# cgranerob/Land-Surface-Temperature-Super-Resolution-with-a-Scale-Invariance-Free-Neural-Approach

Measured on AMD Instinct MI355X. Metric: LST+NDVI 256x256 patches/sec (train fwd+bwd), whole job, higher is better.
Workload: dtype f32; 1 GPU; ModelB SIF-NN-SR2 (gradFTM loss) batch 64/GPU, synthetic 256x256, 1x MI355X, fwd+loss+bwd+Adam; batch_per_gpu=64, patch=256x256 (LST 64x64 + NDVI 256x256), parallelism=dp1, loss=sr2

## Files before the change

land-surface-temperature-super-resolution-with-a-scale-invariance-free-neural-approach_amd/csrc/resample.hip:

```cpp
#include "edge_conv.h"

namespace {

__device__ __forceinline__ float4 maybe_bnrelu(float4 v, const float* scale, const float* shift, int c) {
  return scale != nullptr ? bn_relu4(v, ld4(scale + c), ld4(shift + c)) : v;
}

template <bool HS>
__global__ void bnrelu_pool2_kernel(const float* __restrict__ y, const float* scale, const float* shift,
                                    float* __restrict__ out, int B, int H, int W, int C) {
  const unsigned Q = C / 4, Ho = H / 2, Wo = W / 2;
  const unsigned n = (unsigned)B * Ho * Wo * Q;
  for (unsigned e = blockIdx.x * blockDim.x + threadIdx.x; e < n; e += gridDim.x * blockDim.x) {
    const unsigned p = e / Q;
    const int c = (int)(e - p * Q) * 4;
    const unsigned rr = p / Wo, ox = p - rr * Wo, b = rr / Ho, oy = rr - b * Ho;
    const size_t s = (((size_t)b * H + 2 * oy) * W + 2 * ox) * C + c;
    const float4 v00 = maybe_bnrelu(ldA4<HS>(y, s), scale, shift, c), v01 = maybe_bnrelu(ldA4<HS>(y, s + C), scale, shift, c);
    const float4 v10 = maybe_bnrelu(ldA4<HS>(y, s + (size_t)W * C), scale, shift, c);
    const float4 v11 = maybe_bnrelu(ldA4<HS>(y, s + (size_t)W * C + C), scale, shift, c);
    float4 o;
    o.x = (v00.x + v01.x + v10.x + v11.x) * 0.25f;
    o.y = (v00.y + v01.y + v10.y + v11.y) * 0.25f;
    o.z = (v00.z + v01.z + v10.z + v11.z) * 0.25f;
    o.w = (v00.w + v01.w + v10.w + v11.w) * 0.25f;
    stA4<HS>(out, (size_t)p * C + c, o);
  }
}

template <bool HS>
__global__ void bnrelu_add_kernel(const float* __restrict__ p, const float* __restrict__ y, const float* scale,
                                  const float* shift, float* __restrict__ out, int C, size_t nquads) {
  const unsigned Q = C / 4;
  for (size_t e = (size_t)blockIdx.x * blockDim.x + threadIdx.x; e < nquads; e += (size_t)gridDim.x * blockDim.x) {
    const int c = (int)((unsigned)e % Q) * 4;
    const float4 a = ldA4<HS>(p, e * 4), v = maybe_bnrelu(ldA4<HS>(y, e * 4), scale, shift, c);
    stA4<HS>(out, e * 4, make_float4(a.x + v.x, a.y + v.y, a.z + v.z, a.w + v.w));
  }
}

__device__ __forceinline__ void up_coord(int o, int in, int out, int& i0, int& i1, float& l0, float& l1) {
  const float ratio = out > 1 ? (float)(in - 1) / (float)(out - 1) : 0.f;
  const float src = ratio * (float)o;
  i0 = (int)src;
  i1 = i0 + (i0 < in - 1 ? 1 : 0);
  l1 = src - (float)i0;
  l0 = 1.f - l1;
}

template <bool HS>
__global__ void bnrelu_up2x_kernel(const float* __restrict__ y, const float* scale, const float* shift,
                                   float* __restrict__ out, int B, int Hin, int Win, int C) {
  const int Q = C / 4, Ho = 2 * Hin, Wo = 2 * Win;
  const size_t n = (size_t)B * Ho * Wo * Q;
  for (size_t e = (size_t)blockIdx.x * blockDim.x + threadIdx.x; e < n; e += (size_t)gridDim.x * blockDim.x) {
    const int c = (int)(e % Q) * 4;
    const size_t p = e / Q;
    const int ox = p % Wo, oy = (p / Wo) % Ho, b = p / ((size_t)Wo * Ho);
    int y0, y1, x0, x1; float hy0, hy1, hx0, hx1;
    up_coord(oy, Hin, Ho, y0, y1, hy0, hy1);
    up_coord(ox, Win, Wo, x0, x1, hx0, hx1);
    const size_t base = (size_t)b * Hin * Win * C + c;
    const float4 v00 = maybe_bnrelu(ldA4<HS>(y, base + ((size_t)y0 * Win + x0) * C), scale, shift, c);
    const float4 v01 = maybe_bnrelu(ldA4<HS>(y, base + ((size_t)y0 * Win + x1) * C), scale, shift, c);
    const float4 v10 = maybe_bnrelu(ldA4<HS>(y, base + ((size_t)y1 * Win + x0) * C), scale, shift, c);
    const float4 v11 = maybe_bnrelu(ldA4<HS>(y, base + ((size_t)y1 * Win + x1) * C), scale, shift, c);
    float4 o;
    o.x = hy0 * (hx0 * v00.x + hx1 * v01.x) + hy1 * (hx0 * v10.x + hx1 * v11.x);
    o.y = hy0 * (hx0 * v00.y + hx1 * v01.y) + hy1 * (hx0 * v10.y + hx1 * v11.y);
    o.z = hy0 * (hx0 * v00.z + hx1 * v01.z) + hy1 * (hx0 * v10.z + hx1 * v11.z);
    o.w = hy0 * (hx0 * v00.w + hx1 * v01.w) + hy1 * (hx0 * v10.w + hx1 * v11.w);
    stA4<HS>(out, p * C + c, o);
  }
}

template <bool HS>
__global__ void pool2_bwd_kernel(const float* __restrict__ gp, float* __restrict__ g, int B, int H, int W, int C,
                                 int accumulate) {
  const int Q = C / 4, Ho = H / 2, Wo = W / 2;
  const size_t n = (size_t)B * H * W * Q;
  for (size_t e = (size_t)blockIdx.x * blockDim.x + threadIdx.x; e < n; e += (size_t)gridDim.x * blockDim.x) {
    const int c = (int)(e % Q) * 4;
    const size_t p = e / Q;
    const int x = p % W, yy = (p / W) % H, b = p / ((size_t)W * H);
    const float4 v = ldA4<HS>(gp, (((size_t)b * Ho + yy / 2) * Wo + x / 2) * C + c);
    float4 o = make_float4(0.25f * v.x, 0.25f * v.y, 0.25f * v.z, 0.25f * v.w);
    if (accumulate) {
      const float4 a = ldA4<HS>(g, p * C + c);
      o.x += a.x; o.y += a.y; o.z += a.z; o.w += a.w;
    }
    stA4<HS>(g, p * C + c, o);
  }
}

template <bool HS>
__global__ void up2x_bwd_kernel(const float* __restrict__ gu, float* __restrict__ g, int B, int Hin, int Win, int C) {
  SIFSR_CHAIN_PRIO();
  const int Q = C / 4, Ho = 2 * Hin, Wo = 2 * Win;
  const size_t n = (size_t)B * Hin * Win * Q;
  for (size_t e = (size_t)blockIdx.x * blockDim.x + threadIdx.x; e < n; e += (size_t)gridDim.x * blockDim.x) {
    const int c = (int)(e % Q) * 4;
    const size_t p = e / Q;
    const int ix = p % Win, iy = (p / Win) % Hin, b = p / ((size_t)Win * Hin);
    float wy[5], wx[5];
#pragma unroll
    for (int k = 0; k < 5; ++k) {
      const int oy = 2 * iy - 2 + k, ox = 2 * ix - 2 + k;
      wy[k] = 0.f; wx[k] = 0.f;
      if (oy >= 0 && oy < Ho) {
        int a0, a1; float l0, l1;
        up_coord(oy, Hin, Ho, a0, a1, l0, l1);
        wy[k] = (a0 == iy ? l0 : 0.f) + (a1 == iy ? l1 : 0.f);
      }
      if (ox >= 0 && ox < Wo) {
        int a0, a1; float l0, l1;
        up_coord(ox, Win, Wo, a0, a1, l0, l1);
        wx[k] = (a0 == ix ? l0 : 0.f) + (a1 == ix ? l1 : 0.f);
      }
    }
    float4 acc = make_float4(0.f, 0.f, 0.f, 0.f);
#pragma unroll
    for (int ky = 0; ky < 5; ++ky) {
      if (wy[ky] == 0.f) continue;
      const int oy = 2 * iy - 2 + ky;
#pragma unroll
      for (int kx = 0; kx < 5; ++kx) {
        if (wx[kx] == 0.f) continue;
        const int ox = 2 * ix - 2 + kx;
        const float w = wy[ky] * wx[kx];
        const float4 v = ldA4<HS>(gu, (((size_t)b * Ho + oy) * Wo + ox) * C + c);
        acc.x = fmaf(w, v.x, acc.x); acc.y = fmaf(w, v.y, acc.y); acc.z = fmaf(w, v.z, acc.z); acc.w = fmaf(w, v.w, acc.w);
      }
    }
    stA4<HS>(g, p * C + c, acc);
  }
}

template <int C, bool HS>
__global__ __launch_bounds__(256) void bnrelu_up2x_tile_kernel(const float* __restrict__ y, const float* scale,
                                                               const float* shift, float* __restrict__ out, int Hin,
                                                               int Win) {
  constexpr int Q = C / 4, SR = 10;
  __shared__ float4 src[SR * SR * Q];
  const int tid = threadIdx.x;
  const int Ho = 2 * Hin, Wo = 2 * Win;
  const int ox0 = blockIdx.x * 16, oy0 = blockIdx.y * 16, b = blockIdx.z;
  int sy0, sx0, t1; float f0, f1;
  up_coord(oy0, Hin, Ho, sy0, t1, f0, f1);
  up_coord(ox0, Win, Wo, sx0, t1, f0, f1);
  for (int e = tid; e < SR * SR * Q; e += 256) {
    const int c4 = e % Q, p = e / Q;
    const int py = p / SR, px = p - py * SR;
    const int gy = min(sy0 + py, Hin - 1), gx = min(sx0 + px, Win - 1);
    src[e] = maybe_bnrelu(ldA4<HS>(y, ((size_t)(b * Hin + gy) * Win + gx) * C + 4 * c4), scale, shift, 4 * c4);
  }
  __syncthreads();
  for (int e = tid; e < 256 * Q; e += 256) {
    const int c4 = e % Q, p = e / Q;
    const int oy = oy0 + (p >> 4), ox = ox0 + (p & 15);
    if (oy >= Ho || ox >= Wo) continue;
    int y0, y1, x0, x1; float hy0, hy1, hx0, hx1;
    up_coord(oy, Hin, Ho, y0, y1, hy0, hy1);
    up_coord(ox, Win, Wo, x0, x1, hx0, hx1);
    const float4 v00 = src[((y0 - sy0) * SR + (x0 - sx0)) * Q + c4], v01 = src[((y0 - sy0) * SR + (x1 - sx0)) * Q + c4];
    const float4 v10 = src[((y1 - sy0) * SR + (x0 - sx0)) * Q + c4], v11 = src[((y1 - sy0) * SR + (x1 - sx0)) * Q + c4];
    float4 o;
    o.x = hy0 * (hx0 * v00.x + hx1 * v01.x) + hy1 * (hx0 * v10.x + hx1 * v11.x);
    o.y = hy0 * (hx0 * v00.y + hx1 * v01.y) + hy1 * (hx0 * v10.y + hx1 * v11.y);
    o.z = hy0 * (hx0 * v00.z + hx1 * v01.z) + hy1 * (hx0 * v10.z + hx1 * v11.z);
    o.w = hy0 * (hx0 * v00.w + hx1 * v01.w) + hy1 * (hx0 * v10.w + hx1 * v11.w);
    stA4<HS>(out, ((size_t)(b * Ho + oy) * Wo + ox) * C + 4 * c4, o);
  }
}

template <int C, bool HS>
__global__ __launch_bounds__(256) void up2x_bwd_tile_kernel(const float* __restrict__ gu, float* __restrict__ g, int Hin,
                                                            int Win, const float* __restrict__ bn_y,
                                                            const float* __restrict__ bn_scale,
                                                            const float* __restrict__ bn_shift,
                                                            float* __restrict__ bn_partials) {
  SIFSR_CHAIN_PRIO();
  constexpr int TL = 8, HR = 2 * TL + 3, NCH = C / 16;
  __shared__ float4 hi[HR * HR * 4];
  __shared__ float4 tmp[HR * TL * 4];
  __shared__ float wxs[TL][5], wys[TL][5];
  const int tid = threadIdx.x;
  const int Ho = 2 * Hin, Wo = 2 * Win;
  const int ix0 = blockIdx.x * TL, iy0 = blockIdx.y * TL;
  const int b = blockIdx.z / NCH, ch0 = (blockIdx.z % NCH) * 16;
  if (tid < 2 * TL * 5) {
    const bool isy = tid >= TL * 5;
    const int t = isy ? tid - TL * 5 : tid;
    const int il = t / 5, k = t - il * 5;
    const int i = (isy ? iy0 : ix0) + il, in = isy ? Hin : Win, on = isy ? Ho : Wo;
    const int o = 2 * i - 2 + k;
    float w = 0.f;
    if (i < in && o >= 0 && o < on) {
      int a0, a1; float l0, l1;
      up_coord(o, in, on, a0, a1, l0, l1);
      w = (a0 == i ? l0 : 0.f) + (a1 == i ? l1 : 0.f);
    }
    if (isy) wys[il][k] = w; else wxs[il][k] = w;
  }
  for (int e = tid; e < HR * HR * 4; e += 256) {
    const int q = e & 3, p = e >> 2;
    const int py = p / HR, px = p - py * HR;
    const int oy = 2 * iy0 - 2 + py, ox = 2 * ix0 - 2 + px;
    float4 v = make_float4(0.f, 0.f, 0.f, 0.f);
    if (oy >= 0 && oy < Ho && ox >= 0 && ox < Wo) v = ldA4<HS>(gu, ((size_t)(b * Ho + oy) * Wo + ox) * C + ch0 + 4 * q);
    hi[e] = v;
  }
  __syncthreads();
  for (int e = tid; e < HR * TL * 4; e += 256) {
    const int q = e & 3, p = e >> 2;
    const int py = p / TL, il = p - py * TL;
    float4 acc = make_float4(0.f, 0.f, 0.f, 0.f);
#pragma unroll
    for (int k = 0; k < 5; ++k) {
      const float w = wxs[il][k];
      const float4 v = hi[(py * HR + 2 * il + k) * 4 + q];
      acc.x = fmaf(w, v.x, acc.x); acc.y = fmaf(w, v.y, acc.y); acc.z = fmaf(w, v.z, acc.z); acc.w = fmaf(w, v.w, acc.w);
    }
    tmp[e] = acc;
  }
  __syncthreads();
  {
    const int q = tid & 3, p = tid >> 2;
    const int il_y = p / TL, il_x = p - il_y * TL;
    const int iy = iy0 + il_y, ix = ix0 + il_x;
    float4 acc = make_float4(0.f, 0.f, 0.f, 0.f);
#pragma unroll
    for (int k = 0; k < 5; ++k) {
      const float w = wys[il_y][k];
      const float4 v = tmp[((2 * il_y + k) * TL + il_x) * 4 + q];
      acc.x = fmaf(w, v.x, acc.x); acc.y = fmaf(w, v.y, acc.y); acc.z = fmaf(w, v.z, acc.z); acc.w = fmaf(w, v.w, acc.w);
    }
    const bool in = iy < Hin && ix < Win;
    acc = as_stored4<HS>(acc);
    if (in) stA4<HS>(g, ((size_t)(b * Hin + iy) * Win + ix) * C + ch0 + 4 * q, acc);
    if (bn_partials != nullptr) {
      float4 d1 = make_float4(0.f, 0.f, 0.f, 0.f), d2 = d1;
      if (in) {
        const float4 yv = ldA4<HS>(bn_y, ((size_t)(b * Hin + iy) * Win + ix) * C + ch0 + 4 * q);
        const float4 sc = ld4(bn_scale + ch0 + 4 * q), sh = ld4(bn_shift + ch0 + 4 * q);
        d1.x = fmaf(yv.x, sc.x, sh.x) > 0.f ? acc.x : 0.f; d2.x = d1.x * yv.x;
        d1.y = fmaf(yv.y, sc.y, sh.y) > 0.f ? acc.y : 0.f; d2.y = d1.y * yv.y;
        d1.z = fmaf(yv.z, sc.z, sh.z) > 0.f ? acc.z : 0.f; d2.z = d1.z * yv.z;
        d1.w = fmaf(yv.w, sc.w, sh.w) > 0.f ? acc.w : 0.f; d2.w = d1.w * yv.w;
      }
      float v8[8] = {d1.x, d1.y, d1.z, d1.w, d2.x, d2.y, d2.z, d2.w};
#pragma unroll
      for (int m = 4; m < 64; m <<= 1)
#pragma unroll
        for (int j = 0; j < 8; ++j) v8[j] += __shfl_xor(v8[j], m);
      __syncthreads();
      float* const red = reinterpret_cast<float*>(hi);
      if ((tid & 63) < 4) {
#pragma unroll
        for (int j = 0; j < 8; ++j) red[((tid >> 6) * 4 + (tid & 3)) * 8 + j] = v8[j];
      }
      __syncthreads();
      if (tid < 32) {
        const int qq = tid & 3, r = (tid >> 2) & 3, which = tid >> 4;
        const float sum = (red[(0 * 4 + qq) * 8 + which * 4 + r] + red[(1 * 4 + qq) * 8 + which * 4 + r]) +
                          (red[(2 * 4 + qq) * 8 + which * 4 + r] + red[(3 * 4 + qq) * 8 + which * 4 + r]);
        const size_t row = ((size_t)b * gridDim.y + blockIdx.y) * gridDim.x + blockIdx.x;
        bn_partials[(row * C + ch0 + 4 * qq + r) * 2 + which] = sum;
      }
    }
  }
}

inline int grid_for(size_t n) {
  size_t b = (n + 255) / 256;
  return (int)(b > 16384 ? 16384 : (b < 1 ? 1 : b));
}

}

int launch_bnrelu_pool2(const float* y, const float* scale, const float* shift, float* out, int B, int H, int W, int C, hipStream_t s) {
  if (H % 2 || W % 2 || C % 4 || (size_t)B * H * W * C >= ((size_t)1 << 32)) return SIFSR_ERR_SHAPE;
  if (sifsr_half_storage()) hipLaunchKernelGGL(bnrelu_pool2_kernel<true>, dim3(grid_for((size_t)B * H / 2 * W / 2 * C / 4)), dim3(256), 0, s, y, scale, shift, out, B, H, W, C);
  else hipLaunchKernelGGL(bnrelu_pool2_kernel<false>, dim3(grid_for((size_t)B * H / 2 * W / 2 * C / 4)), dim3(256), 0, s, y, scale, shift, out, B, H, W, C);
  SIFSR_LAUNCH_CHECK();
  return SIFSR_OK;
}
int launch_bnrelu_add(const float* p, const float* y, const float* scale, const float* shift, float* out, int C, size_t npix, hipStream_t s) {
  if (C % 4) return SIFSR_ERR_SHAPE;
  const size_t nq = npix * C / 4;
  if (sifsr_half_storage()) hipLaunchKernelGGL(bnrelu_add_kernel<true>, dim3(grid_for(nq)), dim3(256), 0, s, p, y, scale, shift, out, C, nq);
  else hipLaunchKernelGGL(bnrelu_add_kernel<false>, dim3(grid_for(nq)), dim3(256), 0, s, p, y, scale, shift, out, C, nq);
  SIFSR_LAUNCH_CHECK();
  return SIFSR_OK;
}
int launch_bnrelu_up2x(const float* y, const float* scale, const float* shift, float* out, int B, int Hin, int Win, int C, hipStream_t s) {
  if (C % 4) return SIFSR_ERR_SHAPE;
  if ((C == 16 || C == 32 || C == 64) && B <= 65535 && Hin >= 2 && Win >= 2) {
    const dim3 grid((2 * Win + 15) / 16, (2 * Hin + 15) / 16, B);
#define SIFSR_UP(CV, HV) hipLaunchKernelGGL((bnrelu_up2x_tile_kernel<CV, HV>), grid, dim3(256), 0, s, y, scale, shift, out, Hin, Win)
    const bool hs = sifsr_half_storage();
    if (C == 16) { if (hs) SIFSR_UP(16, true); else SIFSR_UP(16, false); }
    else if (C == 32) { if (hs) SIFSR_UP(32, true); else SIFSR_UP(32, false); }
    else { if (hs) SIFSR_UP(64, true); else SIFSR_UP(64, false); }
#undef SIFSR_UP
    SIFSR_LAUNCH_CHECK();
    return SIFSR_OK;
  }
  if (sifsr_half_storage()) hipLaunchKernelGGL(bnrelu_up2x_kernel<true>, dim3(grid_for((size_t)B * Hin * Win * C)), dim3(256), 0, s, y, scale, shift, out, B, Hin, Win, C);
  else hipLaunchKernelGGL(bnrelu_up2x_kernel<false>, dim3(grid_for((size_t)B * Hin * Win * C)), dim3(256), 0, s, y, scale, shift, out, B, Hin, Win, C);
  SIFSR_LAUNCH_CHECK();
  return SIFSR_OK;
}
int launch_pool2_bwd(const float* gp, float* g, int B, int H, int W, int C, int accumulate, hipStream_t s) {
  if (H % 2 || W % 2 || C % 4) return SIFSR_ERR_SHAPE;
  if (sifsr_half_storage()) hipLaunchKernelGGL(pool2_bwd_kernel<true>, dim3(grid_for((size_t)B * H * W * C / 4)), dim3(256), 0, s, gp, g, B, H, W, C, accumulate);
  else hipLaunchKernelGGL(pool2_bwd_kernel<false>, dim3(grid_for((size_t)B * H * W * C / 4)), dim3(256), 0, s, gp, g, B, H, W, C, accumulate);
  SIFSR_LAUNCH_CHECK();
  return SIFSR_OK;
}
int up2x_bwd_stat_rows(int B, int Hin, int Win, int C) {
  if (!((C == 16 || C == 32 || C == 64) && (size_t)B * (C / 16) <= 65535)) return 0;
  return B * ((Hin + 7) / 8) * ((Win + 7) / 8);
}

int launch_up2x_bwd(const float* gu, float* g, int B, int Hin, int Win, int C, hipStream_t s, const float* bn_y,
                    const float* bn_scale, const float* bn_shift, float* bn_partials) {
  if (C % 4) return SIFSR_ERR_SHAPE;
  if (bn_partials != nullptr && (!bn_y || !bn_scale || !bn_shift || up2x_bwd_stat_rows(B, Hin, Win, C) == 0)) return SIFSR_ERR_ARG;
  if ((C == 16 || C == 32 || C == 64) && (size_t)B * (C / 16) <= 65535) {
    const dim3 grid((Win + 7) / 8, (Hin + 7) / 8, B * (C / 16));
#define SIFSR_UPB(CV, HV) hipLaunchKernelGGL((up2x_bwd_tile_kernel<CV, HV>), grid, dim3(256), 0, s, gu, g, Hin, Win, bn_y, bn_scale, bn_shift, bn_partials)
    const bool hs = sifsr_half_storage();
    if (C == 16) { if (hs) SIFSR_UPB(16, true); else SIFSR_UPB(16, false); }
    else if (C == 32) { if (hs) SIFSR_UPB(32, true); else SIFSR_UPB(32, false); }
    else { if (hs) SIFSR_UPB(64, true); else SIFSR_UPB(64, false); }
#undef SIFSR_UPB
    SIFSR_LAUNCH_CHECK();
    return SIFSR_OK;
  }
  if (sifsr_half_storage()) hipLaunchKernelGGL(up2x_bwd_kernel<true>, dim3(grid_for((size_t)B * Hin * Win * C / 4)), dim3(256), 0, s, gu, g, B, Hin, Win, C);
  else hipLaunchKernelGGL(up2x_bwd_kernel<false>, dim3(grid_for((size_t)B * Hin * Win * C / 4)), dim3(256), 0, s, gu, g, B, Hin, Win, C);
  SIFSR_LAUNCH_CHECK();
  return SIFSR_OK;
}
```

Baseline: 10680 patches/s.

## Replace tiled up2x backward with register-streaming row-band kernel using wave shuffles

Swaps the shared-memory 8x8 tile kernel for the bilinear-upsample backward pass for one that streams output rows down a band of input rows. Each lane keeps its columns in registers, gets horizontal halo neighbours through wave shuffles, and prefetches several rows ahead. It accumulates two vertical input rows as it goes and fuses the BN statistics partials into the same stream. This removes the LDS staging, the block barriers and the redundant halo loads of the tiled version, in exchange for more register pressure and a different grid and partials layout.

```diff
diff --git a/land-surface-temperature-super-resolution-with-a-scale-invariance-free-neural-approach_amd/csrc/resample.hip b/land-surface-temperature-super-resolution-with-a-scale-invariance-free-neural-approach_amd/csrc/resample.hip
--- a/land-surface-temperature-super-resolution-with-a-scale-invariance-free-neural-approach_amd/csrc/resample.hip
+++ b/land-surface-temperature-super-resolution-with-a-scale-invariance-free-neural-approach_amd/csrc/resample.hip
@@ -173,100 +173,137 @@
   }
 }
 
+constexpr int UPB_PF = 3;
+constexpr int upb_band(int C) { return C == 64 ? 8 : 16; }
+
+template <bool HS>
+__device__ __forceinline__ float4 ld_if(bool p, const float* base, size_t e) {
+  return p ? ldA4<HS>(base, e) : make_float4(0.f, 0.f, 0.f, 0.f);
+}
+__device__ __forceinline__ float4 shfl4(float4 v, int src) {
+  return make_float4(__shfl(v.x, src), __shfl(v.y, src), __shfl(v.z, src), __shfl(v.w, src));
+}
+__device__ __forceinline__ float4 sel4(bool p, float4 a, float4 b) { return p ? a : b; }
+__device__ __forceinline__ void fma4(float w, float4 v, float4& acc) {
+  acc.x = fmaf(w, v.x, acc.x); acc.y = fmaf(w, v.y, acc.y); acc.z = fmaf(w, v.z, acc.z); acc.w = fmaf(w, v.w, acc.w);
+}
+__device__ __forceinline__ float up_adj_w(int i, int o, int in, int on) {
+  if (i >= in || o < 2 * i - 2 || o > 2 * i + 2 || o < 0 || o >= on) return 0.f;
+  int a0, a1; float l0, l1;
+  up_coord(o, in, on, a0, a1, l0, l1);
+  return (a0 == i ? l0 : 0.f) + (a1 == i ? l1 : 0.f);
+}
+
 template <int C, bool HS>
-__global__ __launch_bounds__(256) void up2x_bwd_tile_kernel(const float* __restrict__ gu, float* __restrict__ g, int Hin,
-                                                            int Win, const float* __restrict__ bn_y,
-                                                            const float* __restrict__ bn_scale,
-                                                            const float* __restrict__ bn_shift,
-                                                            float* __restrict__ bn_partials) {
+__global__ __launch_bounds__(256) __attribute__((amdgpu_waves_per_eu(4, 8))) void up2x_bwd_stream_kernel(const float* __restrict__ gu, float* __restrict__ g, int Hin,
+                                                              int Win, const float* __restrict__ bn_y,
+                                                              const float* __restrict__ bn_scale,
+                                                              const float* __restrict__ bn_shift,
+                                                              float* __restrict__ bn_partials) {
   SIFSR_CHAIN_PRIO();
-  constexpr int TL = 8, HR = 2 * TL + 3, NCH = C / 16;
-  __shared__ float4 hi[HR * HR * 4];
-  __shared__ float4 tmp[HR * TL * 4];
-  __shared__ float wxs[TL][5], wys[TL][5];
-  const int tid = threadIdx.x;
+  constexpr int Q = C / 4, PW = 64 / Q, PF = UPB_PF, UPB_BAND = upb_band(C);
+  __shared__ float red[4][Q][8];
+  __shared__ float4 bnp[2][Q];
+  const int tid = threadIdx.x, lane = tid & 63, wv = tid >> 6;
+  const int q = lane % Q, pw = lane / Q;
   const int Ho = 2 * Hin, Wo = 2 * Win;
-  const int ix0 = blockIdx.x * TL, iy0 = blockIdx.y * TL;
-  const int b = blockIdx.z / NCH, ch0 = (blockIdx.z % NCH) * 16;
-  if (tid < 2 * TL * 5) {
-    const bool isy = tid >= TL * 5;
-    const int t = isy ? tid - TL * 5 : tid;
-    const int il = t / 5, k = t - il * 5;
-    const int i = (isy ? iy0 : ix0) + il, in = isy ? Hin : Win, on = isy ? Ho : Wo;
-    const int o = 2 * i - 2 + k;
-    float w = 0.f;
-    if (i < in && o >= 0 && o < on) {
-      int a0, a1; float l0, l1;
-      up_coord(o, in, on, a0, a1, l0, l1);
-      w = (a0 == i ? l0 : 0.f) + (a1 == i ? l1 : 0.f);
-    }
-    if (isy) wys[il][k] = w; else wxs[il][k] = w;
-  }
-  for (int e = tid; e < HR * HR * 4; e += 256) {
-    const int q = e & 3, p = e >> 2;
-    const int py = p / HR, px = p - py * HR;
-    const int oy = 2 * iy0 - 2 + py, ox = 2 * ix0 - 2 + px;
-    float4 v = make_float4(0.f, 0.f, 0.f, 0.f);
-    if (oy >= 0 && oy < Ho && ox >= 0 && ox < Wo) v = ldA4<HS>(gu, ((size_t)(b * Ho + oy) * Wo + ox) * C + ch0 + 4 * q);
-    hi[e] = v;
-  }
-  __syncthreads();
-  for (int e = tid; e < HR * TL * 4; e += 256) {
-    const int q = e & 3, p = e >> 2;
-    const int py = p / TL, il = p - py * TL;
-    float4 acc = make_float4(0.f, 0.f, 0.f, 0.f);
-#pragma unroll
-    for (int k = 0; k < 5; ++k) {
-      const float w = wxs[il][k];
-      const float4 v = hi[(py * HR + 2 * il + k) * 4 + q];
-      acc.x = fmaf(w, v.x, acc.x); acc.y = fmaf(w, v.y, acc.y); acc.z = fmaf(w, v.z, acc.z); acc.w = fmaf(w, v.w, acc.w);
-    }
-    tmp[e] = acc;
-  }
-  __syncthreads();
-  {
-    const int q = tid & 3, p = tid >> 2;
-    const int il_y = p / TL, il_x = p - il_y * TL;
-    const int iy = iy0 + il_y, ix = ix0 + il_x;
-    float4 acc = make_float4(0.f, 0.f, 0.f, 0.f);
-#pragma unroll
-    for (int k = 0; k < 5; ++k) {
-      const float w = wys[il_y][k];
-      const float4 v = tmp[((2 * il_y + k) * TL + il_x) * 4 + q];
-      acc.x = fmaf(w, v.x, acc.x); acc.y = fmaf(w, v.y, acc.y); acc.z = fmaf(w, v.z, acc.z); acc.w = fmaf(w, v.w, acc.w);
-    }
-    const bool in = iy < Hin && ix < Win;
+  const int b = blockIdx.z;
+  const int wix0 = (blockIdx.x * 4 + wv) * PW, ix = wix0 + pw;
+  const int r0 = blockIdx.y * UPB_BAND, r1 = min(r0 + UPB_BAND, Hin);
+  const int oy0 = max(2 * r0 - 2, 0), nrows = min(2 * r1, Ho - 1) - oy0 + 1;
+  float wx[5];
+#pragma unroll
+  for (int k = 0; k < 5; ++k) wx[k] = up_adj_w(ix, 2 * ix - 2 + k, Win, Wo);
+  const bool own = ix < Win;
+  const bool first = pw == 0, last = pw == PW - 1;
+  const bool ld_l = last && wix0 > 0 && wix0 < Win;
+  const bool ld_r = first && 2 * (wix0 + PW) < Wo;
+  const bool ld_h = ld_l || ld_r;
+  const int srcl = (lane - Q) & 63, srcr = (lane + Q) & 63;
+  const size_t rowsz = (size_t)Wo * C;
+  const size_t gu_b = (size_t)b * Ho * rowsz, g_b = (size_t)b * Hin * Win * C;
+  const unsigned ca = (unsigned)(2 * ix) * C + 4 * q;
+  const unsigned ch = (unsigned)(ld_l ? 2 * wix0 - 2 : 2 * (wix0 + PW)) * C + 4 * q;
+  const unsigned cg = (unsigned)ix * C + 4 * q;
+
+  float4 va[PF], vb[PF], h0[PF], h1[PF];
+#pragma unroll
+  for (int j = 0; j < PF; ++j) {
+    const size_t ro = gu_b + (size_t)(oy0 + min(j, nrows - 1)) * rowsz;
+    va[j] = ld_if<HS>(own, gu, ro + ca); vb[j] = ld_if<HS>(own, gu, ro + ca + C);
+    h0[j] = ld_if<HS>(ld_h, gu, ro + ch); h1[j] = ld_if<HS>(ld_l, gu, ro + ch + C);
+  }
+
+  const float4 zero = make_float4(0.f, 0.f, 0.f, 0.f);
+  float4 acc_a = zero, acc_b = zero;
+  int cur;
+  { int a1; float l0, l1; up_coord(oy0, Hin, Ho, cur, a1, l0, l1); }
+  const bool stats = bn_partials != nullptr;
+  float4 s1 = zero, s2 = zero, ynext = zero;
+  if (stats) {
+    if (tid < 2 * Q) bnp[tid / Q][tid % Q] = ld4((tid < Q ? bn_scale : bn_shift) + 4 * (tid % Q));
+    __syncthreads();
+    ynext = ld_if<HS>(own, bn_y, g_b + (size_t)r0 * Win * C + cg);
+  }
+  auto flush = [&](int row, float4 acc) {
+    if (row < r0 || row >= r1) return;
     acc = as_stored4<HS>(acc);
-    if (in) stA4<HS>(g, ((size_t)(b * Hin + iy) * Win + ix) * C + ch0 + 4 * q, acc);
-    if (bn_partials != nullptr) {
-      float4 d1 = make_float4(0.f, 0.f, 0.f, 0.f), d2 = d1;
-      if (in) {
-        const float4 yv = ldA4<HS>(bn_y, ((size_t)(b * Hin + iy) * Win + ix) * C + ch0 + 4 * q);
-        const float4 sc = ld4(bn_scale + ch0 + 4 * q), sh = ld4(bn_shift + ch0 + 4 * q);
-        d1.x = fmaf(yv.x, sc.x, sh.x) > 0.f ? acc.x : 0.f; d2.x = d1.x * yv.x;
-        d1.y = fmaf(yv.y, sc.y, sh.y) > 0.f ? acc.y : 0.f; d2.y = d1.y * yv.y;
-        d1.z = fmaf(yv.z, sc.z, sh.z) > 0.f ? acc.z : 0.f; d2.z = d1.z * yv.z;
-        d1.w = fmaf(yv.w, sc.w, sh.w) > 0.f ? acc.w : 0.f; d2.w = d1.w * yv.w;
+    const size_t e = g_b + (size_t)row * Win * C + cg;
+    if (own) stA4<HS>(g, e, acc);
+    if (stats) {
+      const float4 yv = ynext, sc = bnp[0][q], sh = bnp[1][q];
+      ynext = ld_if<HS>(own && row + 1 < r1, bn_y, e + (size_t)Win * C);
+      float d;
+      d = fmaf(yv.x, sc.x, sh.x) > 0.f ? acc.x : 0.f; s1.x += d; s2.x = fmaf(d, yv.x, s2.x);
+      d = fmaf(yv.y, sc.y, sh.y) > 0.f ? acc.y : 0.f; s1.y += d; s2.y = fmaf(d, yv.y, s2.y);
+      d = fmaf(yv.z, sc.z, sh.z) > 0.f ? acc.z : 0.f; s1.z += d; s2.z = fmaf(d, yv.z, s2.z);
+      d = fmaf(yv.w, sc.w, sh.w) > 0.f ? acc.w : 0.f; s1.w += d; s2.w = fmaf(d, yv.w, s2.w);
+    }
+  };
+
+  for (int base = 0; base < nrows; base += PF) {
+#pragma unroll
+    for (int j = 0; j < PF; ++j) {
+      const int r = base + j;
+      if (r >= nrows) break;
+      const int oy = oy0 + r;
+      const float4 a = va[j], bb = vb[j];
+      const float4 l2 = shfl4(sel4(last, h0[j], a), srcl), l1 = shfl4(sel4(last, h1[j], bb), srcl);
+      const float4 rr = shfl4(sel4(first, h0[j], a), srcr);
+      if (r + PF < nrows) {
+        const size_t ro = gu_b + (size_t)(oy + PF) * rowsz;
+        va[j] = ld_if<HS>(own, gu, ro + ca); vb[j] = ld_if<HS>(own, gu, ro + ca + C);
+        h0[j] = ld_if<HS>(ld_h, gu, ro + ch); h1[j] = ld_if<HS>(ld_l, gu, ro + ch + C);
       }
-      float v8[8] = {d1.x, d1.y, d1.z, d1.w, d2.x, d2.y, d2.z, d2.w};
-#pragma unroll
-      for (int m = 4; m < 64; m <<= 1)
-#pragma unroll
-        for (int j = 0; j < 8; ++j) v8[j] += __shfl_xor(v8[j], m);
-      __syncthreads();
-      float* const red = reinterpret_cast<float*>(hi);
-      if ((tid & 63) < 4) {
-#pragma unroll
-        for (int j = 0; j < 8; ++j) red[((tid >> 6) * 4 + (tid & 3)) * 8 + j] = v8[j];
-      }
-      __syncthreads();
-      if (tid < 32) {
-        const int qq = tid & 3, r = (tid >> 2) & 3, which = tid >> 4;
-        const float sum = (red[(0 * 4 + qq) * 8 + which * 4 + r] + red[(1 * 4 + qq) * 8 + which * 4 + r]) +
-                          (red[(2 * 4 + qq) * 8 + which * 4 + r] + red[(3 * 4 + qq) * 8 + which * 4 + r]);
-        const size_t row = ((size_t)b * gridDim.y + blockIdx.y) * gridDim.x + blockIdx.x;
-        bn_partials[(row * C + ch0 + 4 * qq + r) * 2 + which] = sum;
-      }
+      float4 h = zero;
+      fma4(wx[0], l2, h); fma4(wx[1], l1, h); fma4(wx[2], a, h); fma4(wx[3], bb, h); fma4(wx[4], rr, h);
+      int a0, a1; float l0f, l1f;
+      up_coord(oy, Hin, Ho, a0, a1, l0f, l1f);
+      if (cur < a0) { flush(cur, acc_a); acc_a = acc_b; acc_b = zero; ++cur; }
+      fma4(up_adj_w(cur, oy, Hin, Ho), h, acc_a);
+      fma4(up_adj_w(cur + 1, oy, Hin, Ho), h, acc_b);
+    }
+  }
+  flush(cur, acc_a);
+  flush(cur + 1, acc_b);
+
+  if (stats) {
+    float v8[8] = {s1.x, s1.y, s1.z, s1.w, s2.x, s2.y, s2.z, s2.w};
+#pragma unroll
+    for (int m = Q; m < 64; m <<= 1)
+#pragma unroll
+      for (int j = 0; j < 8; ++j) v8[j] += __shfl_xor(v8[j], m);
+    if (lane < Q) {
+#pragma unroll
+      for (int j = 0; j < 8; ++j) red[wv][lane][j] = v8[j];
+    }
+    __syncthreads();
+    if (tid < 2 * C) {
+      const int which = tid & 1, c = tid >> 1;
+      const int k = which * 4 + (c & 3);
+      const float sum = (red[0][c >> 2][k] + red[1][c >> 2][k]) + (red[2][c >> 2][k] + red[3][c >> 2][k]);
+      const size_t row = ((size_t)b * gridDim.y + blockIdx.y) * gridDim.x + blockIdx.x;
+      bn_partials[(row * C + c) * 2 + which] = sum;
     }
   }
 }
@@ -318,18 +355,23 @@
   SIFSR_LAUNCH_CHECK();
   return SIFSR_OK;
 }
+static bool up2x_bwd_streams(int B, int Hin, int Win, int C) {
+  return (C == 16 || C == 32 || C == 64) && B >= 1 && B <= 65535 && Hin >= 2 && Win >= 2 &&
+         (Hin + upb_band(C) - 1) / upb_band(C) <= 65535 && (size_t)2 * Win * C < ((size_t)1 << 31);
+}
 int up2x_bwd_stat_rows(int B, int Hin, int Win, int C) {
-  if (!((C == 16 || C == 32 || C == 64) && (size_t)B * (C / 16) <= 65535)) return 0;
-  return B * ((Hin + 7) / 8) * ((Win + 7) / 8);
+  if (!up2x_bwd_streams(B, Hin, Win, C)) return 0;
+  const size_t rows = (size_t)B * ((Hin + upb_band(C) - 1) / upb_band(C)) * ((Win + 1024 / C - 1) / (1024 / C));
+  return rows <= 0x7fffffff ? (int)rows : 0;
 }
 
 int launch_up2x_bwd(const float* gu, float* g, int B, int Hin, int Win, int C, hipStream_t s, const float* bn_y,
                     const float* bn_scale, const float* bn_shift, float* bn_partials) {
   if (C % 4) return SIFSR_ERR_SHAPE;
   if (bn_partials != nullptr && (!bn_y || !bn_scale || !bn_shift || up2x_bwd_stat_rows(B, Hin, Win, C) == 0)) return SIFSR_ERR_ARG;
-  if ((C == 16 || C == 32 || C == 64) && (size_t)B * (C / 16) <= 65535) {
-    const dim3 grid((Win + 7) / 8, (Hin + 7) / 8, B * (C / 16));
-#define SIFSR_UPB(CV, HV) hipLaunchKernelGGL((up2x_bwd_tile_kernel<CV, HV>), grid, dim3(256), 0, s, gu, g, Hin, Win, bn_y, bn_scale, bn_shift, bn_partials)
+  if (up2x_bwd_streams(B, Hin, Win, C)) {
+    const dim3 grid((Win + 1024 / C - 1) / (1024 / C), (Hin + upb_band(C) - 1) / upb_band(C), B);
+#define SIFSR_UPB(CV, HV) hipLaunchKernelGGL((up2x_bwd_stream_kernel<CV, HV>), grid, dim3(256), 0, s, gu, g, Hin, Win, bn_y, bn_scale, bn_shift, bn_partials)
     const bool hs = sifsr_half_storage();
     if (C == 16) { if (hs) SIFSR_UPB(16, true); else SIFSR_UPB(16, false); }
     else if (C == 32) { if (hs) SIFSR_UPB(32, true); else SIFSR_UPB(32, false); }
```

Measured after the change: 10760 patches/s (median of 6 runs). No clear change (+0.8%).
